# steineggerlab/unicore

Hardware: AMD Instinct MI355X
Metric: 3Di alignments/sec (cluster path) (higher is better)
Workload: dtype u16

## Files before the change

unicore_amd/csrc/uc_prefilter.hip:

```cpp
#include <hip/hip_runtime.h>

#include <algorithm>
#include <cstdlib>
#include <cstring>
#include <type_traits>

#include <rocprim/rocprim.hpp>

#include "uc_engine.h"

namespace uc {

constexpr uint32_t KMER_INVALID = 0xFFFFFFFFu;

struct KmerCfg {
    int koff[K];
    int span;
    int thr;
};

__device__ __forceinline__ uint32_t find_seq(const uint32_t *off, uint32_t lo, uint32_t hi, uint32_t p) {
    while (hi - lo > 1) {
        const uint32_t mid = lo + ((hi - lo) >> 1);
        if (off[mid] <= p) lo = mid; else hi = mid;
// ... 51 lines not shown
        bits[w] = m;
    }
}

constexpr int SIM_NEED_MAX = 49;
struct SimTables {
    int8_t sc[KA][KA];
    uint8_t ord[KA][KA];
    int8_t rowmax[KA];
    uint8_t lcnt[KA][2 * SIM_NEED_MAX + 1];
    uint32_t pmask[KA][KA + 1];
};

__device__ void build_sim_tables(SimTables &t, const int8_t *S3) {
    for (int a = threadIdx.x; a < KA; a += blockDim.x) {
        int8_t sc[KA];
        uint8_t ord[KA];
        for (int b = 0; b < KA; b++) { sc[b] = S3[a * 21 + b]; ord[b] = (uint8_t)b; }
        for (int i = 1; i < KA; i++) {
            const int8_t s = sc[i];
            const uint8_t o = ord[i];
            int k = i - 1;
            while (k >= 0 && (sc[k] < s)) { sc[k + 1] = sc[k]; ord[k + 1] = ord[k]; k--; }
            sc[k + 1] = s;
            ord[k + 1] = o;
        }
        for (int b = 0; b < KA; b++) { t.sc[a][b] = sc[b]; t.ord[a][b] = ord[b]; }
        t.rowmax[a] = sc[0];
    }
    for (int i = threadIdx.x; i < KA * (2 * SIM_NEED_MAX + 1); i += blockDim.x) {
        const int a = i / (2 * SIM_NEED_MAX + 1), need = i % (2 * SIM_NEED_MAX + 1) - SIM_NEED_MAX;
        int n = 0;
        for (int b = 0; b < KA; b++) n += S3[a * 21 + b] >= need ? 1 : 0;
        t.lcnt[a][i % (2 * SIM_NEED_MAX + 1)] = (uint8_t)n;
    }
    __syncthreads();
    for (int i = threadIdx.x; i < KA * (KA + 1); i += blockDim.x) {
        const int a = i / (KA + 1), n = i % (KA + 1);
        uint32_t m = 0;
        for (int j = 0; j < n; j++) m |= 1u << t.ord[a][j];
        t.pmask[a][n] = m;
    }
// ... 1 lines not shown

__device__ __forceinline__ bool query_kmer_at(const DeviceDb &db, const KmerCfg &cfg, uint32_t qbegin, uint32_t qend,
                                              uint32_t p, uint32_t *q, uint32_t *i, uint32_t c[K]) {
    const uint32_t s = find_seq(db.off, qbegin, qend, p);
    const uint32_t j = p - db.off[s], len = db.len[s];
    *q = s;
    *i = j;
    if (!(j + cfg.span <= len && j <= 65535u)) return false;
    bool ok = true;
#pragma unroll
    for (int m = 0; m < K; m++) { c[m] = db.s3[p + cfg.koff[m]]; ok &= c[m] < KA; }
    return ok;
}

constexpr int RUN_STAGE = 256;

struct RunList {
    uint32_t *pidx;
    uint64_t *val;
    uint64_t cap;
};

constexpr int LEAFQ = 256;
constexpr int POSQ = 128;
constexpr int SIM_MIN_WAVE_POS = 256;
constexpr int SIM_MAX_BLOCKS = 1024;

__global__ void __launch_bounds__(256) sim_runs_kernel(const DeviceDb db, KmerCfg cfg, uint32_t qbegin, uint32_t qend,
                                                            uint32_t p0, uint32_t p1, const uint32_t *koff, RunList out,
                                                            unsigned long long *counters,
                                                            const uint32_t *dk ,
                                                            uint32_t *nsim_k ,
                                                            uint32_t item_stride ,
                                                            const uint32_t *kbits = nullptr ) {
    __shared__ SimTables tab;
    __shared__ uint32_t s_mul[K];
    __shared__ uint32_t s_n[4];
    __shared__ uint64_t s_val[4][RUN_STAGE];
    __shared__ uint32_t s_pi[4][RUN_STAGE];
    __shared__ uint32_t s_qv[4][LEAFQ], s_qp[4][LEAFQ], s_qm[4][LEAFQ];
    __shared__ uint32_t s_pc[4][POSQ], s_pp[4][POSQ];
    __shared__ uint64_t s_pr[4][POSQ];
    build_sim_tables(tab, db.S3);
    const int wv = threadIdx.x >> 6, lane = threadIdx.x & 63;
    if (threadIdx.x < K) { uint32_t m = 1; for (int i = 0; i < K - 1 - (int)threadIdx.x; i++) m *= KA; s_mul[threadIdx.x] = m; }
    if (lane == 0) s_n[wv] = 0;
    __syncthreads();
    volatile uint32_t *vn = &s_n[wv];
    volatile uint64_t *vval = s_val[wv];
    volatile uint32_t *vpi = s_pi[wv];
    volatile uint32_t *qv = s_qv[wv], *qp = s_qp[wv], *qm = s_qm[wv];
    volatile uint32_t *pc = s_pc[wv], *pp = s_pp[wv];
    volatile uint64_t *pr = s_pr[wv];
    const int thr = cfg.thr, thrb = thr + 256;

    auto flush_runs = [&]() {
        const uint32_t n = *vn;
        uint32_t blo = 0, bhi = 0;
        if (lane == 0) {
            const unsigned long long b = atomicAdd(counters + 3, (unsigned long long)n);
            blo = (uint32_t)b; bhi = (uint32_t)(b >> 32);
        }
        blo = (uint32_t)__shfl((int)blo, 0, 64);
        bhi = (uint32_t)__shfl((int)bhi, 0, 64);
        const uint64_t base = ((uint64_t)bhi << 32) | blo;
        for (uint32_t k = lane; k < n; k += 64) {
            const uint64_t w = base + k;
            if (w < out.cap) { out.pidx[w] = vpi[k]; out.val[w] = vval[k]; }
        }
        __builtin_amdgcn_wave_barrier();
        if (lane == 0) *vn = 0;
        __builtin_amdgcn_wave_barrier();
    };
    unsigned long long nhit = 0;
    auto drain_leaves = [&](uint32_t qn) {
        for (uint32_t b = 0; b < qn; b += 64) {
            const uint32_t i = b + lane;
            uint32_t m = 0, v0 = 0, pi = 0;
            if (i < qn) {
                v0 = qv[i]; pi = qp[i]; m = qm[i];
                if (kbits) {
                    const uint32_t w = v0 >> 5, sh = v0 & 31;
                    const uint64_t two = (uint64_t)kbits[w] | ((uint64_t)(sh > 32 - KA ? kbits[w + 1] : 0u) << 32);
// ... 136 lines not shown
            }
            const uint64_t lm = __builtin_amdgcn_ballot_w64(leaf);
            if (lm) {
                if (leaf) { const uint32_t slot = qn + (uint32_t)__popcll(lm & ((1ull << lane) - 1ull)); qv[slot] = leafv; qp[slot] = pidx; qm[slot] = leafm; }
                qn += (uint32_t)__popcll(lm);
                nsim += (unsigned long long)__popc(leafm);
                if (qn > LEAFQ - 64) { __builtin_amdgcn_wave_barrier(); drain_leaves(qn); qn = 0; }
            }
        }
        __builtin_amdgcn_wave_barrier();
        drain_leaves(qn);
        if (nsim_k && has_item) nsim_k[pidx] = lc;
    }
    __builtin_amdgcn_wave_barrier();
    flush_runs();
    for (int o = 32; o > 0; o >>= 1) { nsim += __shfl_down(nsim, o, 64); nhit += __shfl_down(nhit, o, 64); }
    if (lane == 0) {
        if (nsim) atomicAdd(counters + 0, nsim);
        if (nhit) atomicAdd(counters + 4, nhit);
    }
}

__global__ void __launch_bounds__(256) query_kmer_kernel(const DeviceDb db, KmerCfg cfg, uint32_t qbegin, uint32_t qend, uint32_t p0, uint32_t p1,
                                                         uint32_t *qk, uint8_t *flag) {
    for (uint64_t idx = (uint64_t)blockIdx.x * 256 + threadIdx.x; idx < p1 - p0; idx += (uint64_t)gridDim.x * 256) {
        uint32_t q, i, c[K];
        uint32_t key = KMER_INVALID;
        if (query_kmer_at(db, cfg, qbegin, qend, p0 + (uint32_t)idx, &q, &i, c)) {
            uint32_t v = 0, mul = 1;
#pragma unroll
            for (int m = 0; m < K; m++) { v += c[m] * mul; mul *= KA; }
            key = v;
            flag[v] = 1;
// ... 170 lines not shown
        const uint32_t want = db.off[qbegin + i] - p0;
        uint64_t lo = 0, hi = n_runs;
        while (lo < hi) { const uint64_t m = (lo + hi) >> 1; if (rpidx[m] < want) lo = m + 1; else hi = m; }
        qr[i] = lo;
    }
}

__global__ void __launch_bounds__(256) run_order_key_kernel(uint32_t nq, const uint64_t *qr, uint32_t *key, uint32_t *idx) {
    for (uint32_t i = blockIdx.x * 256 + threadIdx.x; i < nq; i += gridDim.x * 256) {
        const uint64_t c = qr[i + 1] - qr[i];
        key[i] = 0xFFFFFFFFu - (uint32_t)min<uint64_t>(c, 0xFFFFFFFFull);
        idx[i] = i;
    }
}

template <bool C> struct TdType { using type = uint64_t; };
template <> struct TdType<true> { using type = uint32_t; };

template <bool C>
__global__ void __launch_bounds__(FT) filter_kernel(const DeviceDb db, uint32_t qbegin, uint32_t p0, const uint32_t *rpidx,
                                                    const uint64_t *rval, const uint64_t *qr, const uint32_t *order, const void *ent, KeyFmt fmt,
                                                    unsigned long long *region_cursor, void *region_v, uint64_t region_cap,
                                                    uint64_t *qbase, uint32_t *qsurv) {
    using TD = typename TdType<C>::type;
    struct __attribute__((aligned(4))) TD4 { TD v[KPT]; };
    TD *region = (TD *)region_v;
    extern __shared__ __attribute__((aligned(16))) uint32_t f_lds[];
    constexpr int BW = 1 << (FB_LOG2 - 5);
    constexpr int RPT = FILTER_RPT;
    constexpr int TR = RPT * FT;
    uint32_t *B1 = f_lds, *B2 = f_lds + BW;
    uint2 *s_run = (uint2 *)(f_lds + 2 * BW);
    uint32_t *s_pref = (uint32_t *)(s_run + TR);
    uint32_t *s_wsum = s_pref + TR + 1;
    uint64_t *s_misc = (uint64_t *)(((uintptr_t)(s_wsum + 16) + 7) & ~(uintptr_t)7);
    const int tid = threadIdx.x, lane = tid & 63, wv = tid >> 6;
    const uint32_t qi = order[blockIdx.x];
// ... 82 lines not shown
    };
    auto mark1 = [&](uint64_t td) {
        uint32_t g;
        const uint32_t h = slot_of(td, g), bit = 1u << (h & 31), gbit = 1u << (g & 31);
        const uint32_t old = atomicOr(&B1[h >> 5], bit);
        if (old & bit) atomicOr(&B2[h >> 5], bit);
        const uint32_t gold = atomicOr(&B1[g >> 5], gbit);
        if (gold & gbit) atomicOr(&B2[g >> 5], gbit);
    };
    auto twice1 = [&](uint64_t td) -> uint32_t {
        uint32_t g;
        const uint32_t h = slot_of(td, g);
        return ((B2[h >> 5] >> (h & 31)) & (B2[g >> 5] >> (g & 31))) & 1u;
    };

    {
        uint64_t part = 0;
        for (uint64_t r = r0 + tid; r < r1; r += FT) part += rval[r] >> 32;
        for (int o = 32; o > 0; o >>= 1) part += __shfl_down(part, o, 64);
        uint64_t *s_part = (uint64_t *)s_pref;
        if (lane == 0) s_part[wv] = part;
        __syncthreads();
        if (tid == 0) {
            uint64_t tot = 0;
            for (int w = 0; w < FT / 64; w++) tot += s_part[w];
            s_misc[2] = atomicAdd(region_cursor, (unsigned long long)((tot + KPT - 1) / KPT * KPT));
            ((uint32_t *)&s_misc[3])[0] = 0;
            ((uint32_t *)&s_misc[3])[1] = 0;
        }
        __syncthreads();
    }
    const uint64_t base = s_misc[2];
    uint32_t *cur = (uint32_t *)&s_misc[3];
    uint32_t total = 0;
    prefetch_tile(r0);
    for (uint64_t tile = r0; tile < r1; tile += TR) {
        load_tile(tile);
        prefetch_tile(tile + TR);
        const uint32_t T = s_pref[TR];
        using ET = typename std::conditional<C, uint32_t, uint64_t>::type;
        auto mark_store = [&](TD4 &td, int n, uint32_t k4) {
#pragma unroll
            for (int i = 0; i < KPT; i++) {
                if (i >= n) { td.v[i] = td.v[0]; continue; }
                mark1(td.v[i]);
            }
            const uint64_t w = base + total + k4;
            if (n && w + KPT <= region_cap) {
                if (n == KPT) *(TD4 *)(region + w) = td;
                else {
#pragma unroll
                    for (int i = 0; i < KPT; i++) if (i < n) region[w + i] = td.v[i];
                }
            }
        };
        for (uint32_t k4 = (uint32_t)KPT * tid; k4 < T; k4 += 2u * KPT * FT) {
            const uint32_t k4b = k4 + (uint32_t)KPT * FT;
            uint32_t ia[KPT], ib[KPT];
            int32_t sa[KPT], sb[KPT];
            const int na = locate(k4, T, ia, sa);
            const int nb = locate(k4b < T ? k4b : k4, T, ib, sb);
            ET ea[KPT], eb[KPT];
            gather(ia, ea);
            gather(ib, eb);
            TD4 ta, tb;
            to_td(ea, sa, ta.v);
            mark_store(ta, na, k4);
            to_td(eb, sb, tb.v);
            mark_store(tb, k4b < T ? nb : 0, k4b);
        }
        total += T;
        __syncthreads();
    }
    __threadfence_block();
    __syncthreads();
    const uint32_t n0 = (uint32_t)min<uint64_t>(total, region_cap > base ? region_cap - base : 0);
    const uint32_t n0r = n0;
    for (uint32_t k4 = (uint32_t)KPT * tid; k4 < n0r; k4 += 2u * KPT * FT) {
        TD4 td[2] = {};
        int nn[2];
#pragma unroll
        for (int g2 = 0; g2 < 2; g2++) {
            const uint32_t k = k4 + (uint32_t)g2 * KPT * FT;
            nn[g2] = k >= n0 ? 0 : (n0 - k < (uint32_t)KPT ? (int)(n0 - k) : KPT);
            if (nn[g2] == KPT) td[g2] = *(const TD4 *)(region + base + k);
            else {
#pragma unroll
                for (int i = 0; i < KPT; i++) if (i < nn[g2]) td[g2].v[i] = region[base + k + i];
            }
        }
        uint32_t keep = 0;
// ... 553 lines not shown
        }
    }
}
__global__ void __launch_bounds__(256) owner_gather_kernel(uint64_t n, const uint32_t *idx, const uint32_t *hq, const uint32_t *ht, const int32_t *hs,
                                                           const int32_t *hd, uint32_t *oq, uint32_t *ot, int32_t *os, int32_t *od) {
    for (uint64_t i = (uint64_t)blockIdx.x * 256 + threadIdx.x; i < n; i += (uint64_t)gridDim.x * 256) {
        const uint32_t j = idx[i];
        oq[i] = hq[j]; ot[i] = ht[j]; os[i] = hs[j]; od[i] = hd[j];
    }
}

struct WidenU32 {
    __host__ __device__ uint64_t operator()(uint32_t x) const { return (uint64_t)x; }
};

struct PrefilterScratch {
    DevBuf<unsigned long long> d_counters;
    DevBuf<char> d_temp;
    DevBuf<uint32_t> d_koff, k_in, k_out, d_ent32, v_in32, d_okey, d_okey2, d_oidx, d_order;
    DevBuf<uint64_t> d_ent, v_in;
    DevBuf<uint32_t> d_cnt, d_flag, d_cq, d_ct, d_rpidx2, d_qsurv;
    DevBuf<uint32_t> d_qcand, d_qmir, d_qrec;
    DevBuf<uint64_t> d_coff;
    DevBuf<uint64_t> d_keys, d_keys2, d_pos, d_skey, d_skey2, d_rval2, d_qbase, d_soff, d_qr;
    DevBuf<int32_t> d_cd, d_cd2, d_score, d_mval;
    DevBuf<uint64_t> d_mkey;
    DevBuf<uint32_t> acc_q, acc_t, pass_q, pass_t;
    DevBuf<int32_t> acc_s, acc_d, pass_s, pass_d;
    DevBuf<uint8_t> d_kflag, d_wflag;
    DevBuf<uint32_t> d_qk, d_kid, d_dk, d_nsimk, d_drk, d_drk2, d_roff, d_nr, d_src, d_ph;
    DevBuf<uint64_t> d_drv, d_drv2, d_cumh, d_cumr, d_qh, d_qrn;
    DevBuf<RankRec> d_rec;
    DevBuf<uint32_t> d_kbits;
    UngappedAllWork ua;
    template <class F> void each(F f) {
        f(d_counters); f(d_temp); f(d_koff); f(k_in); f(k_out); f(d_ent32); f(v_in32); f(d_okey); f(d_okey2); f(d_oidx); f(d_order);
        f(d_ent); f(v_in); f(d_cnt); f(d_flag); f(d_cq); f(d_ct); f(d_rpidx2); f(d_qsurv); f(d_keys); f(d_keys2); f(d_pos); f(d_skey);
        f(d_skey2); f(d_rval2); f(d_qbase); f(d_soff); f(d_qr); f(d_cd); f(d_cd2); f(d_score); f(d_kflag); f(d_wflag); f(d_qk); f(d_kid); f(d_dk);
        f(d_nsimk); f(d_drk); f(d_drk2); f(d_roff); f(d_nr); f(d_src); f(d_ph); f(d_drv); f(d_drv2); f(d_cumh); f(d_cumr); f(d_qh); f(d_qrn); f(d_rec); f(d_kbits); f(d_mkey); f(d_mval); f(acc_q); f(acc_t); f(pass_q); f(pass_t); f(acc_s); f(acc_d); f(pass_s); f(pass_d);
        f(d_qcand); f(d_qmir); f(d_qrec); f(d_coff); f(ua.score); f(ua.diag); f(ua.pairs); f(ua.prof); f(ua.prof_off);
    }
    size_t bytes() {
        size_t b = 0;
        each([&](auto &x) { b += x.cap * sizeof(*x.p); });
        return b;
    }
    void release_bytes(size_t target) {
        if (getenv("UC_TIMING")) {
            fprintf(stderr, "unicore-cluster[timing]: prefilter scratch %.1f GiB, %.1f GiB to give back before the gapped stage; buffers >= 2 GiB (index in PrefilterScratch::each: GiB):", bytes() / 1073741824.0, target / 1073741824.0);
            int i = 0;
            each([&](auto &x) { const double g = x.cap * sizeof(*x.p) / 1073741824.0; if (g >= 2.0) fprintf(stderr, " %d:%.1f", i, g); i++; });
            fprintf(stderr, "\n");
        }
        if (!target) return;
        if (target >= bytes()) { each([&](auto &x) { if (x.cap * sizeof(*x.p) >= ((size_t)1 << 30)) x.release(); }); return; }
// ... 45 lines not shown
    if (hit_off[n] != n_hits) fail(UC_ERR_GENERIC, "%s: hit list bookkeeping mismatch", who);
}

constexpr uint64_t RUN_MAX = 1ull << 29;
struct PrefilterPass {
    KmerCfg cfg;
    KeyFmt fmt;
    uint32_t tbegin = 0, tend = 0;
    uint32_t qbegin = 0, qend = 0;
    uint32_t mirror_q0 = UINT32_MAX;
    bool count_sims = false;
    double density_limit = 0.0, *density_out = nullptr;
    const void *ent_p = nullptr;
    uint32_t n_entries = 0;
    uint64_t HIT_CAP = 0, HIT_CAP_BIG = 0, DRUN_MAX = 0;
    uint64_t td_queries = 0, td_keys = 0, filt_queries = 0, filt_keys = 0;
    uint32_t td_cap = 0;
    uint64_t n_hits_total = 0, n_cand_total = 0, cand_cap = 0, run_cap = 1ull << 20;
    double t_kmer = 0, t_ung = 0, t_sel = 0, gpu_ms = 0;
};
struct SuperBatch {
    uint32_t begin = 0, end = 0;
    uint32_t P0 = 0, NP = 0;
    std::vector<uint64_t> h_qh, h_qr;
    uint64_t hit_cap = 0;
    double frac = 1.0;
};
struct QueryBatch {
    uint32_t qa = 0, qb = 0;
    uint64_t total_hits = 0, n_runs = 0;
// ... 43 lines not shown
    S.d_kbits.reserve((KSPACE + 31) / 32);
    hipLaunchKernelGGL(kmer_bits_kernel, grid_for((KSPACE + 31) / 32), dim3(256), 0, E.stream, (const uint32_t *)S.d_koff.p, S.d_kbits.p);
    UC_HIP(hipMemcpyAsync(&PP.n_entries, S.d_koff.p + KSPACE, 4, hipMemcpyDeviceToHost, E.stream));
    UC_HIP(hipStreamSynchronize(E.stream));
    UC_HIP(hipGetLastError());
    PP.gpu_ms = E.timed_ms_end();
    E.stats.n_index_entries += PP.n_entries;
    E.stats.algorithmic_bytes[UC_ST_INDEX] += 6ull * PP.n_entries + 8ull * KSPACE;
    E.stats.stage_seconds[UC_ST_INDEX] += t_index.seconds();
}

static dim3 sim_grid(uint64_t items) {
    return dim3((uint32_t)std::min<uint64_t>(std::max<uint64_t>(1, (items + 4 * SIM_MIN_WAVE_POS - 1) / (4 * SIM_MIN_WAVE_POS)), SIM_MAX_BLOCKS));
}

static uint64_t distinct_runs(Engine &E, PrefilterPass &PP, const SuperBatch &SB, uint32_t nd, uint64_t &n_druns, uint64_t &drun_cap) {
    PrefilterScratch &S = *E.pre;
    const uint32_t nqa = SB.end - SB.begin;
    if (nqa > 1 && nd > (1u << 16)) {
        const uint32_t st = 64;
        UC_HIP(hipMemsetAsync(S.d_counters.p + 3, 0, 32, E.stream));
        UC_HIP(hipMemsetAsync(S.d_counters.p, 0, 8, E.stream));
        hipLaunchKernelGGL(sim_runs_kernel, sim_grid((nd + st - 1) / st), dim3(256), 0, E.stream, E.ddb, PP.cfg, 0u, 0u, 0u, nd, S.d_koff.p, RunList{nullptr, nullptr, 0},
                           S.d_counters.p, S.d_dk.p, (uint32_t *)nullptr, st, (const uint32_t *)S.d_kbits.p);
        unsigned long long c5[5];
        UC_HIP(hipMemcpyAsync(c5, S.d_counters.p, 40, hipMemcpyDeviceToHost, E.stream));
        UC_HIP(hipStreamSynchronize(E.stream));
        if ((double)c5[3] * st > 0.9 * (double)PP.DRUN_MAX) return (uint64_t)((double)c5[3] * st / 0.9);
    }
    n_druns = 0; drun_cap = S.d_drk.cap;
    for (;;) {
        drun_cap = std::min<uint64_t>(1ull << 32, std::max<uint64_t>(drun_cap, std::max<uint64_t>(1u << 20, std::min<uint64_t>(PP.DRUN_MAX, (uint64_t)nd * 16))));
        S.d_drk.reserve(drun_cap); S.d_drv.reserve(drun_cap);
        UC_HIP(hipMemsetAsync(S.d_counters.p + 3, 0, 32, E.stream));
        UC_HIP(hipMemsetAsync(S.d_counters.p, 0, 8, E.stream));
        const RunList rl{S.d_drk.p, S.d_drv.p, drun_cap};
        hipLaunchKernelGGL(sim_runs_kernel, sim_grid(nd), dim3(256), 0, E.stream, E.ddb, PP.cfg, 0u, 0u, 0u, nd, S.d_koff.p, rl, S.d_counters.p, S.d_dk.p, S.d_nsimk.p, 1u,
                           (const uint32_t *)S.d_kbits.p);
        unsigned long long c5[5];
        UC_HIP(hipMemcpyAsync(c5, S.d_counters.p, 40, hipMemcpyDeviceToHost, E.stream));
        UC_HIP(hipStreamSynchronize(E.stream));
        n_druns = c5[3];
        if (getenv("UC_TIMING")) fprintf(stderr, "unicore-cluster[timing]: similar k-mers of %u distinct k-mers: %llu index runs\n", nd, (unsigned long long)n_druns);
        if (n_druns > PP.DRUN_MAX && nqa > 1) return n_druns;
        if (n_druns > drun_cap) {
            if (n_druns >= (1ull << 32)) fail(UC_ERR_GENERIC, "%u distinct k-mers of query %u produce %llu index ranges", nd, SB.begin, (unsigned long long)n_druns);
            drun_cap = n_druns;
            UC_HIP(hipMemsetAsync(S.d_nsimk.p, 0, (size_t)std::max<uint32_t>(nd, 1) * 4, E.stream));
            continue;
        }
        return 0;
    }
}

enum class PlanStatus { planned, too_dense , too_many_runs  };
struct PlanResult { PlanStatus status; uint64_t over_runs; };
static PlanResult plan_superbatch(Engine &E, PrefilterPass &PP, SuperBatch &SB, uint32_t sa, uint32_t sb) {
    PrefilterScratch &S = *E.pre;
    uint64_t plan_hits = 0;
    SB.begin = sa; SB.end = sb;
    SB.P0 = E.h_poff[sa]; SB.NP = E.h_poff[sb] - SB.P0;
    const uint32_t NP = SB.NP, nqa = sb - sa;
    Timer t_p;
    E.timed_ms_begin();
    S.d_qk.reserve((size_t)NP + 1); S.d_kflag.reserve((size_t)KSPACE + 1); S.d_kid.reserve((size_t)KSPACE + 1);
    UC_HIP(hipMemsetAsync(S.d_kflag.p, 0, (size_t)KSPACE + 1, E.stream));
    hipLaunchKernelGGL(query_kmer_kernel, grid_for(NP), dim3(256), 0, E.stream, E.ddb, PP.cfg, sa, sb, SB.P0, SB.P0 + NP, S.d_qk.p, S.d_kflag.p);
    auto fin = rocprim::make_transform_iterator(S.d_kflag.p, FlagToU32());
    rocprim_call(S.d_temp, [&](void *t, size_t &b) { return rocprim::exclusive_scan(t, b, fin, S.d_kid.p, 0u, (size_t)KSPACE + 1, rocprim::plus<uint32_t>(), E.stream); });
    uint32_t nd = 0;
    UC_HIP(hipMemcpyAsync(&nd, S.d_kid.p + KSPACE, 4, hipMemcpyDeviceToHost, E.stream));
    UC_HIP(hipStreamSynchronize(E.stream));
    S.d_dk.reserve(std::max<uint32_t>(nd, 1)); S.d_nsimk.reserve(std::max<uint32_t>(nd, 1));
    UC_HIP(hipMemsetAsync(S.d_nsimk.p, 0, (size_t)std::max<uint32_t>(nd, 1) * 4, E.stream));
    hipLaunchKernelGGL(distinct_kmer_kernel, grid_for(KSPACE), dim3(256), 0, E.stream, S.d_kflag.p, S.d_kid.p, S.d_dk.p);
    uint64_t n_druns = 0, drun_cap = 0;
    if (const uint64_t over_runs = distinct_runs(E, PP, SB, nd, n_druns, drun_cap)) {
        PP.gpu_ms += E.timed_ms_end();
        PP.t_kmer += t_p.seconds();
        return {PlanStatus::too_many_runs, over_runs};
    }
    unsigned dbits = 1;
    while ((1ull << dbits) < nd) dbits++;
    S.d_drk2.reserve(drun_cap); S.d_drv2.reserve(drun_cap);
    if (n_druns)
        rocprim_call(S.d_temp, [&](void *t, size_t &b) { return rocprim::radix_sort_pairs(t, b, S.d_drk.p, S.d_drk2.p, S.d_drv.p, S.d_drv2.p, (size_t)n_druns, 0u, dbits, E.stream); });
    S.d_roff.reserve((size_t)nd + 1); S.d_rec.reserve(std::max<uint32_t>(nd, 1));
    hipLaunchKernelGGL(rank_offsets_kernel, grid_for((uint64_t)nd + 1), dim3(256), 0, E.stream, S.d_drk2.p, (uint32_t)n_druns, nd, S.d_roff.p);
    if (nd) hipLaunchKernelGGL(rank_rec_kernel, grid_for(nd), dim3(256), 0, E.stream, S.d_roff.p, S.d_drv2.p, S.d_nsimk.p, nd, S.d_rec.p);
    S.d_nr.reserve((size_t)NP + 1); S.d_src.reserve((size_t)NP + 1); S.d_ph.reserve((size_t)NP + 1);
    S.d_cumh.reserve((size_t)NP + 1); S.d_cumr.reserve((size_t)NP + 1);
    UC_HIP(hipMemsetAsync(S.d_counters.p, 0, 8, E.stream));
    UC_HIP(hipMemsetAsync(S.d_nr.p + NP, 0, 4, E.stream));
    UC_HIP(hipMemsetAsync(S.d_ph.p + NP, 0, 4, E.stream));
    hipLaunchKernelGGL(position_runs_kernel, grid_for(NP, E.count_grid_cap), dim3(256), 0, E.stream, S.d_qk.p, NP, S.d_kid.p, S.d_rec.p, S.d_nr.p, S.d_src.p, S.d_ph.p, S.d_counters.p);
    auto hin = rocprim::make_transform_iterator(S.d_ph.p, WidenU32());
    auto rin = rocprim::make_transform_iterator(S.d_nr.p, WidenU32());
    rocprim_call(S.d_temp, [&](void *t, size_t &b) { return rocprim::exclusive_scan(t, b, hin, S.d_cumh.p, (uint64_t)0, (size_t)NP + 1, rocprim::plus<uint64_t>(), E.stream); });
    rocprim_call(S.d_temp, [&](void *t, size_t &b) { return rocprim::exclusive_scan(t, b, rin, S.d_cumr.p, (uint64_t)0, (size_t)NP + 1, rocprim::plus<uint64_t>(), E.stream); });
    S.d_qh.reserve(nqa); S.d_qrn.reserve(nqa);
    hipLaunchKernelGGL(query_totals_kernel, grid_for(nqa), dim3(256), 0, E.stream, E.ddb.off, sa, nqa, SB.P0, S.d_cumh.p, S.d_cumr.p, S.d_qh.p, S.d_qrn.p);
// ... 63 lines not shown
    B.kbits = (unsigned)(PP.fmt.dbits + PP.fmt.tbits) + qbits;
    return B;
}

static uint64_t compact_u64(Engine &E, DevBuf<char> &tmp, uint32_t *cnt, uint64_t *pos, uint64_t n, const uint32_t *also = nullptr, uint32_t *also_out = nullptr) {
    auto in = rocprim::make_transform_iterator(cnt, WidenU32());
    rocprim_call(tmp, [&](void *t, size_t &b) { return rocprim::exclusive_scan(t, b, in, pos, (uint64_t)0, (size_t)n, rocprim::plus<uint64_t>(), E.stream); });
    uint64_t lp = 0; uint32_t lc = 0;
    UC_HIP(hipMemcpyAsync(&lp, pos + (n - 1), 8, hipMemcpyDeviceToHost, E.stream));
    UC_HIP(hipMemcpyAsync(&lc, cnt + (n - 1), 4, hipMemcpyDeviceToHost, E.stream));
    if (also) UC_HIP(hipMemcpyAsync(also_out, also, 4, hipMemcpyDeviceToHost, E.stream));
    UC_HIP(hipStreamSynchronize(E.stream));
    return lp + lc;
}

static void expand_keys_filtered(Engine &E, PrefilterPass &PP, QueryBatch &B) {
    PrefilterScratch &S = *E.pre;
    const KeyFmt &fmt = PP.fmt;
    const uint32_t qa = B.qa, qp0 = B.qp0, nq = B.qb - B.qa;
    S.d_qbase.reserve(nq); S.d_qsurv.reserve(nq); S.d_soff.reserve((size_t)nq + 1);
    const uint64_t region_cap = B.total_hits + (uint64_t)KPT * nq;
    S.d_keys.reserve(fmt.compact ? region_cap : 2 * region_cap);
    S.d_qr.reserve((size_t)nq + 1);
    hipLaunchKernelGGL(run_range_kernel, grid_for((uint64_t)nq + 1), dim3(256), 0, E.stream, E.ddb, qa, nq, qp0, S.d_rpidx2.p, B.n_runs, S.d_qr.p);
    S.d_okey.reserve(nq); S.d_okey2.reserve(nq); S.d_oidx.reserve(nq); S.d_order.reserve(nq);
    hipLaunchKernelGGL(run_order_key_kernel, grid_for(nq), dim3(256), 0, E.stream, nq, S.d_qr.p, S.d_okey.p, S.d_oidx.p);
    rocprim_call(S.d_temp, [&](void *t, size_t &b) { return rocprim::radix_sort_pairs(t, b, S.d_okey.p, S.d_okey2.p, S.d_oidx.p, S.d_order.p, (size_t)nq, 0u, 32u, E.stream); });
    auto launch = [&](auto kern) {
        static PerDeviceOnce once[2];
        once[fmt.compact ? 1 : 0]([&] { UC_HIP(hipFuncSetAttribute((const void *)kern, hipFuncAttributeMaxDynamicSharedMemorySize, (int)filter_lds(FILTER_RPT))); });
        hipLaunchKernelGGL(kern, dim3(nq), dim3(FT), filter_lds(FILTER_RPT), E.stream, E.ddb, qa, qp0, S.d_rpidx2.p, S.d_rval2.p, S.d_qr.p, S.d_order.p, PP.ent_p, fmt,
                           S.d_counters.p + 5, (void *)S.d_keys.p, region_cap, S.d_qbase.p, S.d_qsurv.p);
    };
    if (fmt.compact) launch(filter_kernel<true>);
    else launch(filter_kernel<false>);
    unsigned long long taken = 0;
    uint32_t last_rec = 0;
    const bool onchip = fmt.compact && PP.td_cap > 0;
    if (onchip) {
        int rbits = 1;
        while ((1ull << rbits) < (uint64_t)std::max<uint32_t>(PP.tend - PP.tbegin, 1)) rbits++;
        S.d_qcand.reserve(nq); S.d_qmir.reserve(nq); S.d_qrec.reserve(nq); S.d_coff.reserve(nq);
        UC_HIP(hipMemsetAsync(S.d_counters.p + 7, 0, 8, E.stream));
        hipLaunchKernelGGL(td_select_kernel<false>, dim3(nq), dim3(TDS_T), 0, E.stream, (uint32_t *)S.d_keys.p, S.d_qbase.p, S.d_qsurv.p, S.d_order.p, qa, PP.mirror_q0,
                           E.p.min_diag_hits, fmt.dbits, (unsigned)std::min(32, rbits + fmt.dbits), PP.td_cap, S.d_qcand.p, S.d_qmir.p, S.d_qrec.p, S.d_counters.p + 7);
        if (PP.td_cap > (uint32_t)TDS_SMALL_IPT * TDS_T)
            hipLaunchKernelGGL(td_select_kernel<true>, dim3(nq), dim3(TDS_T), 0, E.stream, (uint32_t *)S.d_keys.p, S.d_qbase.p, S.d_qsurv.p, S.d_order.p, qa, PP.mirror_q0,
// ... 117 lines not shown

static bool prefilter_one(Engine &E, uint32_t tbegin, uint32_t tend, uint32_t qbegin, uint32_t qend, bool count_sims, double density_limit,
                          double *density_out, uint32_t mirror_q0) {
    UC_HIP(hipSetDevice(E.device));
    const uint32_t n = E.hdb.n;
    PrefilterPass PP;
    for (int m = 0; m < K; m++) PP.cfg.koff[m] = E.p.koff[m];
    PP.cfg.span = E.p.span; PP.cfg.thr = E.p.kmer_thr;
    PP.tbegin = tbegin; PP.tend = tend; PP.qbegin = qbegin; PP.qend = qend; PP.mirror_q0 = mirror_q0;
    PP.count_sims = count_sims; PP.density_limit = density_limit; PP.density_out = density_out;
    const char *hc = getenv("UC_HIT_CAP");
    PP.HIT_CAP = hc ? std::max<uint64_t>(1u << 20, strtoull(hc, nullptr, 10)) : (3ull << 29);
    PP.HIT_CAP_BIG = hc ? PP.HIT_CAP : (15ull << 28);
    const char *dm = getenv("UC_DRUN_MAX");
    PP.DRUN_MAX = dm ? std::max<uint64_t>(1, strtoull(dm, nullptr, 10)) : (1ull << 31);
    const char *to = getenv("UC_TD_ONCHIP"), *tc = getenv("UC_TD_ONCHIP_CAP");
    PP.td_cap = to && atoi(to) == 0 ? 0u : TDS_CAP;
    if (PP.td_cap && tc) {
        const uint64_t want = strtoull(tc, nullptr, 10);
        uint32_t c = 64;
        while (c < TDS_CAP && 2ull * c <= want) c *= 2;
        PP.td_cap = c;
    }

    E.hit_cnt.assign(n, 0);
    E.hit_off.assign((size_t)n + 1, 0);
    E.n_hits = 0;
    E.alns_valid = false;
    E.clear_edges();
    const uint64_t sims_before = E.stats.n_sim_kmers;

    if (n > (1u << 24)) fail(UC_ERR_GENERIC, "prefilter: %u sequences exceed the 2^24 limit of the hit keys", n);
    if (!E.pre) E.pre = ParkedScratch<PrefilterScratch>::take_or_new(E.device);
    E.pre->d_counters.reserve(8);
    UC_HIP(hipMemsetAsync(E.pre->d_counters.p, 0, 64, E.stream));

    build_index(E, PP);
    SuperBatch SB;
    SB.begin = SB.end = qbegin;
    for (uint32_t qa = qbegin; qa < qend;) {
        if (qa >= SB.end && !choose_superbatch(E, PP, SB, qa)) return false;
        Timer t_b;
        E.timed_ms_begin();
        QueryBatch B = cut_batch(E, PP, SB, qa);
        uint64_t n_cand = 0;
        if (B.total_hits) {
            if (E.p.min_diag_hits >= 2 && B.total_hits < (1ull << 32)) expand_keys_filtered(E, PP, B);
            else expand_keys_plain(E, PP, B);
            n_cand = select_diagonals(E, PP, B);
        }
        UC_HIP(hipGetLastError());
        PP.gpu_ms += E.timed_ms_end();
        PP.t_kmer += t_b.seconds();
        PP.n_cand_total += n_cand;
        if (n_cand) {
            rescore_ungapped(E, PP, n_cand);
            select_and_append(E, PP, n_cand);
        }
        qa = B.qb;
    }
    finish_chunk(E, PP, sims_before);
    return true;
// ... 20 lines not shown
            acc_n = E.merge_hits_dev(acc_n, S.acc_q.p, S.acc_t.p, S.acc_s.p, S.acc_d.p, n_pass, S.pass_q.p, S.pass_t.p, S.pass_s.p, S.pass_d.p, !mir, 0, 1);
            if (c + 1 == chunks.size()) installed = true;
            else swap_acc();
        }
    }
    if (!installed) E.merge_hits_dev(acc_n, S.acc_q.p, S.acc_t.p, S.acc_s.p, S.acc_d.p, 0, nullptr, nullptr, nullptr, nullptr, true, 0, 1);
    return true;
}

static void prefilter_exhaustive(Engine &E, uint32_t tbegin, uint32_t tend, uint32_t qbegin, uint32_t qend) {
    UC_HIP(hipSetDevice(E.device));
    if (E.hdb.n > (1u << 24)) fail(UC_ERR_GENERIC, "prefilter: %u sequences exceed the 2^24 limit of the hit keys", E.hdb.n);
    logf(3, "unicore-cluster: --prefilter-mode 1: all %u x %u pairs are scored on every diagonal; --k-score, --min-diag-hits and -s have no effect\n", qend - qbegin, tend - tbegin);
    if (!E.pre) E.pre = ParkedScratch<PrefilterScratch>::take_or_new(E.device);
    PrefilterScratch &S = *E.pre;
    S.d_counters.reserve(8);
    UC_HIP(hipMemsetAsync(S.d_counters.p, 0, 64, E.stream));
    uint64_t budget = UNGAPPED_ALL_TILE_BYTES;
    if (const char *ev = getenv("UC_UNGAPPED_TILE_BYTES")) budget = std::max<uint64_t>(1, strtoull(ev, nullptr, 10));
    uint32_t QB = 1, TC = 1;
    ungapped_all_plan(budget, qend - qbegin, tend - tbegin, &QB, &TC);
    UngappedAllWork &W = S.ua;
    PrefilterPass PP;
    bool installed = false;
    const auto swap_acc = [&] { swap_hits(E, S.acc_q, S.acc_t, S.acc_s, S.acc_d); };
    uint64_t acc_n = 0, cells = 0;
    for (uint32_t qa = qbegin; qa < qend; qa += std::min(QB, qend - qa))
        for (uint32_t ta = tbegin; ta < tend; ta += std::min(TC, tend - ta)) {
            const uint32_t nq = std::min(QB, qend - qa), nt = std::min(TC, tend - ta);
            const uint64_t np = (uint64_t)nq * nt;
            Timer t_u;
            E.timed_ms_begin();
// ... 246 lines not shown
```

Baseline: 23.05 million.

## Reserve run slots in per-wave chunks and precompute filter region bases by scan

sim_runs_kernel now reserves output slots for similar-k-mer runs in fixed-size chunks per wave instead of one global atomic per flush, and pads unused chunk tails with sentinel entries. Run and nsim counts are moved to separate counters, and the sort uses the extended slot count. filter_kernel no longer does a block reduction plus a global atomic to claim its region; base offsets come from an exclusive scan over per-query hit counts. This cuts contention on global atomics, at the cost of larger run buffers and extra padding entries to sort.

```diff
diff --git a/unicore_amd/csrc/uc_prefilter.hip b/unicore_amd/csrc/uc_prefilter.hip
--- a/unicore_amd/csrc/uc_prefilter.hip
+++ b/unicore_amd/csrc/uc_prefilter.hip
@@ -89,8 +89,8 @@
 
 __device__ void build_sim_tables(SimTables &t, const int8_t *S3) {
     for (int a = threadIdx.x; a < KA; a += blockDim.x) {
-        int8_t sc[KA];
-        uint8_t ord[KA];
+        int8_t *sc = t.sc[a];
+        uint8_t *ord = t.ord[a];
         for (int b = 0; b < KA; b++) { sc[b] = S3[a * 21 + b]; ord[b] = (uint8_t)b; }
         for (int i = 1; i < KA; i++) {
             const int8_t s = sc[i];
@@ -100,7 +100,6 @@
             sc[k + 1] = s;
             ord[k + 1] = o;
         }
-        for (int b = 0; b < KA; b++) { t.sc[a][b] = sc[b]; t.ord[a][b] = ord[b]; }
         t.rowmax[a] = sc[0];
     }
     for (int i = threadIdx.x; i < KA * (2 * SIM_NEED_MAX + 1); i += blockDim.x) {
@@ -132,6 +131,7 @@
 }
 
 constexpr int RUN_STAGE = 256;
+constexpr uint32_t RUN_CHUNK = 2048;
 
 struct RunList {
     uint32_t *pidx;
@@ -150,6 +150,7 @@
                                                             const uint32_t *dk ,
                                                             uint32_t *nsim_k ,
                                                             uint32_t item_stride ,
+                                                            uint32_t run_chunk ,
                                                             const uint32_t *kbits = nullptr ) {
     __shared__ SimTables tab;
     __shared__ uint32_t s_mul[K];
@@ -172,19 +173,30 @@
     volatile uint64_t *pr = s_pr[wv];
     const int thr = cfg.thr, thrb = thr + 256;
 
+    uint64_t cpos = 0, cend = 0, nruns = 0;
     auto flush_runs = [&]() {
-        const uint32_t n = *vn;
-        uint32_t blo = 0, bhi = 0;
-        if (lane == 0) {
-            const unsigned long long b = atomicAdd(counters + 3, (unsigned long long)n);
-            blo = (uint32_t)b; bhi = (uint32_t)(b >> 32);
-        }
-        blo = (uint32_t)__shfl((int)blo, 0, 64);
-        bhi = (uint32_t)__shfl((int)bhi, 0, 64);
-        const uint64_t base = ((uint64_t)bhi << 32) | blo;
-        for (uint32_t k = lane; k < n; k += 64) {
-            const uint64_t w = base + k;
-            if (w < out.cap) { out.pidx[w] = vpi[k]; out.val[w] = vval[k]; }
+        const uint32_t n = (uint32_t)__builtin_amdgcn_readfirstlane((int)*vn);
+        nruns += n;
+        if (out.pidx) {
+            for (uint32_t k0 = 0; k0 < n;) {
+                if (cpos == cend) {
+                    uint32_t blo = 0, bhi = 0;
+                    if (lane == 0) {
+                        const unsigned long long b = atomicAdd(counters + 8, (unsigned long long)run_chunk);
+                        blo = (uint32_t)b; bhi = (uint32_t)(b >> 32);
+                    }
+                    blo = (uint32_t)__builtin_amdgcn_readfirstlane((int)blo);
+                    bhi = (uint32_t)__builtin_amdgcn_readfirstlane((int)bhi);
+                    cpos = ((uint64_t)bhi << 32) | blo;
+                    cend = cpos + run_chunk;
+                }
+                const uint32_t m = (uint32_t)min((uint64_t)(n - k0), cend - cpos);
+                for (uint32_t k = lane; k < m; k += 64) {
+                    const uint64_t w = cpos + k;
+                    if (w < out.cap) { out.pidx[w] = vpi[k0 + k]; out.val[w] = vval[k0 + k]; }
+                }
+                cpos += m; k0 += m;
+            }
         }
         __builtin_amdgcn_wave_barrier();
         if (lane == 0) *vn = 0;
@@ -351,9 +363,11 @@
     }
     __builtin_amdgcn_wave_barrier();
     flush_runs();
+    for (uint64_t w = cpos + lane; w < min(cend, out.cap); w += 64) { out.pidx[w] = p1 - p0; out.val[w] = 0; }
     for (int o = 32; o > 0; o >>= 1) { nsim += __shfl_down(nsim, o, 64); nhit += __shfl_down(nhit, o, 64); }
     if (lane == 0) {
-        if (nsim) atomicAdd(counters + 0, nsim);
+        if (nruns) atomicAdd(counters + 3, (unsigned long long)nruns);
+        if (nsim) atomicAdd(counters + 9, nsim);
         if (nhit) atomicAdd(counters + 4, nhit);
     }
 }
@@ -554,13 +568,18 @@
     }
 }
 
+struct RoundUpKpt {
+    __host__ __device__ uint64_t operator()(uint64_t h) const { return (h + KPT - 1) / KPT * KPT; }
+};
+
 template <bool C> struct TdType { using type = uint64_t; };
 template <> struct TdType<true> { using type = uint32_t; };
 
 template <bool C>
 __global__ void __launch_bounds__(FT) filter_kernel(const DeviceDb db, uint32_t qbegin, uint32_t p0, const uint32_t *rpidx,
                                                     const uint64_t *rval, const uint64_t *qr, const uint32_t *order, const void *ent, KeyFmt fmt,
-                                                    unsigned long long *region_cursor, void *region_v, uint64_t region_cap,
+                                                    const uint64_t *rbase ,
+                                                    const uint64_t *qhits , void *region_v, uint64_t region_cap,
                                                     uint64_t *qbase, uint32_t *qsurv) {
     using TD = typename TdType<C>::type;
     struct __attribute__((aligned(4))) TD4 { TD v[KPT]; };
@@ -673,24 +692,10 @@
         return ((B2[h >> 5] >> (h & 31)) & (B2[g >> 5] >> (g & 31))) & 1u;
     };
 
-    {
-        uint64_t part = 0;
-        for (uint64_t r = r0 + tid; r < r1; r += FT) part += rval[r] >> 32;
-        for (int o = 32; o > 0; o >>= 1) part += __shfl_down(part, o, 64);
-        uint64_t *s_part = (uint64_t *)s_pref;
-        if (lane == 0) s_part[wv] = part;
-        __syncthreads();
-        if (tid == 0) {
-            uint64_t tot = 0;
-            for (int w = 0; w < FT / 64; w++) tot += s_part[w];
-            s_misc[2] = atomicAdd(region_cursor, (unsigned long long)((tot + KPT - 1) / KPT * KPT));
-            ((uint32_t *)&s_misc[3])[0] = 0;
-            ((uint32_t *)&s_misc[3])[1] = 0;
-        }
-        __syncthreads();
-    }
-    const uint64_t base = s_misc[2];
+    const uint64_t base = rbase[qi];
+    const uint64_t region_end = min(base + (qhits[qi] + KPT - 1) / KPT * KPT, region_cap);
     uint32_t *cur = (uint32_t *)&s_misc[3];
+    if (tid == 0) { cur[0] = 0; cur[1] = 0; }
     uint32_t total = 0;
     prefetch_tile(r0);
     for (uint64_t tile = r0; tile < r1; tile += TR) {
@@ -705,7 +710,7 @@
                 mark1(td.v[i]);
             }
             const uint64_t w = base + total + k4;
-            if (n && w + KPT <= region_cap) {
+            if (n && w + n <= region_end) {
                 if (n == KPT) *(TD4 *)(region + w) = td;
                 else {
 #pragma unroll
@@ -733,7 +738,7 @@
     }
     __threadfence_block();
     __syncthreads();
-    const uint32_t n0 = (uint32_t)min<uint64_t>(total, region_cap > base ? region_cap - base : 0);
+    const uint32_t n0 = (uint32_t)min<uint64_t>(total, region_end > base ? region_end - base : 0);
     const uint32_t n0r = n0;
     for (uint32_t k4 = (uint32_t)KPT * tid; k4 < n0r; k4 += 2u * KPT * FT) {
         TD4 td[2] = {};
@@ -1317,6 +1322,7 @@
     __host__ __device__ uint64_t operator()(uint32_t x) const { return (uint64_t)x; }
 };
 
+constexpr size_t PREFILTER_COUNTERS = 10;
 struct PrefilterScratch {
     DevBuf<unsigned long long> d_counters;
     DevBuf<char> d_temp;
@@ -1325,7 +1331,7 @@
     DevBuf<uint32_t> d_cnt, d_flag, d_cq, d_ct, d_rpidx2, d_qsurv;
     DevBuf<uint32_t> d_qcand, d_qmir, d_qrec;
     DevBuf<uint64_t> d_coff;
-    DevBuf<uint64_t> d_keys, d_keys2, d_pos, d_skey, d_skey2, d_rval2, d_qbase, d_soff, d_qr;
+    DevBuf<uint64_t> d_keys, d_keys2, d_pos, d_skey, d_skey2, d_rval2, d_qbase, d_soff, d_qr, d_rbase;
     DevBuf<int32_t> d_cd, d_cd2, d_score, d_mval;
     DevBuf<uint64_t> d_mkey;
     DevBuf<uint32_t> acc_q, acc_t, pass_q, pass_t;
@@ -1341,7 +1347,7 @@
         f(d_ent); f(v_in); f(d_cnt); f(d_flag); f(d_cq); f(d_ct); f(d_rpidx2); f(d_qsurv); f(d_keys); f(d_keys2); f(d_pos); f(d_skey);
         f(d_skey2); f(d_rval2); f(d_qbase); f(d_soff); f(d_qr); f(d_cd); f(d_cd2); f(d_score); f(d_kflag); f(d_wflag); f(d_qk); f(d_kid); f(d_dk);
         f(d_nsimk); f(d_drk); f(d_drk2); f(d_roff); f(d_nr); f(d_src); f(d_ph); f(d_drv); f(d_drv2); f(d_cumh); f(d_cumr); f(d_qh); f(d_qrn); f(d_rec); f(d_kbits); f(d_mkey); f(d_mval); f(acc_q); f(acc_t); f(pass_q); f(pass_t); f(acc_s); f(acc_d); f(pass_s); f(pass_d);
-        f(d_qcand); f(d_qmir); f(d_qrec); f(d_coff); f(ua.score); f(ua.diag); f(ua.pairs); f(ua.prof); f(ua.prof_off);
+        f(d_qcand); f(d_qmir); f(d_qrec); f(d_coff); f(d_rbase); f(ua.score); f(ua.diag); f(ua.pairs); f(ua.prof); f(ua.prof_off);
     }
     size_t bytes() {
         size_t b = 0;
@@ -1417,6 +1423,8 @@
     const void *ent_p = nullptr;
     uint32_t n_entries = 0;
     uint64_t HIT_CAP = 0, HIT_CAP_BIG = 0, DRUN_MAX = 0;
+    uint64_t DRUN_CAP0 = 0;
+    uint32_t run_chunk = RUN_CHUNK;
     uint64_t td_queries = 0, td_keys = 0, filt_queries = 0, filt_keys = 0;
     uint32_t td_cap = 0;
     uint64_t n_hits_total = 0, n_cand_total = 0, cand_cap = 0, run_cap = 1ull << 20;
@@ -1490,38 +1498,42 @@
     return dim3((uint32_t)std::min<uint64_t>(std::max<uint64_t>(1, (items + 4 * SIM_MIN_WAVE_POS - 1) / (4 * SIM_MIN_WAVE_POS)), SIM_MAX_BLOCKS));
 }
 
-static uint64_t distinct_runs(Engine &E, PrefilterPass &PP, const SuperBatch &SB, uint32_t nd, uint64_t &n_druns, uint64_t &drun_cap) {
+static uint64_t distinct_runs(Engine &E, PrefilterPass &PP, const SuperBatch &SB, uint32_t nd, uint64_t &n_druns, uint64_t &n_ext, uint64_t &drun_cap) {
     PrefilterScratch &S = *E.pre;
     const uint32_t nqa = SB.end - SB.begin;
+    unsigned long long c[6];
     if (nqa > 1 && nd > (1u << 16)) {
         const uint32_t st = 64;
-        UC_HIP(hipMemsetAsync(S.d_counters.p + 3, 0, 32, E.stream));
-        UC_HIP(hipMemsetAsync(S.d_counters.p, 0, 8, E.stream));
+        UC_HIP(hipMemsetAsync(S.d_counters.p + 3, 0, 56, E.stream));
         hipLaunchKernelGGL(sim_runs_kernel, sim_grid((nd + st - 1) / st), dim3(256), 0, E.stream, E.ddb, PP.cfg, 0u, 0u, 0u, nd, S.d_koff.p, RunList{nullptr, nullptr, 0},
-                           S.d_counters.p, S.d_dk.p, (uint32_t *)nullptr, st, (const uint32_t *)S.d_kbits.p);
-        unsigned long long c5[5];
-        UC_HIP(hipMemcpyAsync(c5, S.d_counters.p, 40, hipMemcpyDeviceToHost, E.stream));
+                           S.d_counters.p, S.d_dk.p, (uint32_t *)nullptr, st, PP.run_chunk, (const uint32_t *)S.d_kbits.p);
+        UC_HIP(hipMemcpyAsync(c, S.d_counters.p + 3, 8, hipMemcpyDeviceToHost, E.stream));
         UC_HIP(hipStreamSynchronize(E.stream));
-        if ((double)c5[3] * st > 0.9 * (double)PP.DRUN_MAX) return (uint64_t)((double)c5[3] * st / 0.9);
-    }
-    n_druns = 0; drun_cap = S.d_drk.cap;
+        if ((double)c[0] * st > 0.9 * (double)PP.DRUN_MAX) return (uint64_t)((double)c[0] * st / 0.9);
+    }
+    const dim3 grid = sim_grid(nd);
+    const uint64_t tails = (uint64_t)grid.x * 4 * PP.run_chunk;
+    n_druns = n_ext = 0;
+    drun_cap = PP.DRUN_CAP0 ? PP.DRUN_CAP0
+                            : std::max<uint64_t>(S.d_drk.cap, std::max<uint64_t>(1u << 20, std::min<uint64_t>(PP.DRUN_MAX, (uint64_t)nd * 16) + tails));
     for (;;) {
-        drun_cap = std::min<uint64_t>(1ull << 32, std::max<uint64_t>(drun_cap, std::max<uint64_t>(1u << 20, std::min<uint64_t>(PP.DRUN_MAX, (uint64_t)nd * 16))));
+        drun_cap = std::min<uint64_t>(1ull << 32, drun_cap);
         S.d_drk.reserve(drun_cap); S.d_drv.reserve(drun_cap);
-        UC_HIP(hipMemsetAsync(S.d_counters.p + 3, 0, 32, E.stream));
-        UC_HIP(hipMemsetAsync(S.d_counters.p, 0, 8, E.stream));
+        UC_HIP(hipMemsetAsync(S.d_counters.p + 3, 0, 56, E.stream));
         const RunList rl{S.d_drk.p, S.d_drv.p, drun_cap};
-        hipLaunchKernelGGL(sim_runs_kernel, sim_grid(nd), dim3(256), 0, E.stream, E.ddb, PP.cfg, 0u, 0u, 0u, nd, S.d_koff.p, rl, S.d_counters.p, S.d_dk.p, S.d_nsimk.p, 1u,
-                           (const uint32_t *)S.d_kbits.p);
-        unsigned long long c5[5];
-        UC_HIP(hipMemcpyAsync(c5, S.d_counters.p, 40, hipMemcpyDeviceToHost, E.stream));
+        hipLaunchKernelGGL(sim_runs_kernel, grid, dim3(256), 0, E.stream, E.ddb, PP.cfg, 0u, 0u, 0u, nd, S.d_koff.p, rl, S.d_counters.p, S.d_dk.p, S.d_nsimk.p, 1u,
+                           PP.run_chunk, (const uint32_t *)S.d_kbits.p);
+        UC_HIP(hipMemcpyAsync(c, S.d_counters.p + 3, 48, hipMemcpyDeviceToHost, E.stream));
         UC_HIP(hipStreamSynchronize(E.stream));
-        n_druns = c5[3];
-        if (getenv("UC_TIMING")) fprintf(stderr, "unicore-cluster[timing]: similar k-mers of %u distinct k-mers: %llu index runs\n", nd, (unsigned long long)n_druns);
+        n_druns = c[0]; n_ext = c[5];
+        if (getenv("UC_TIMING"))
+            fprintf(stderr, "unicore-cluster[timing]: similar k-mers of %u distinct k-mers: %llu index runs in %llu reserved slots (capacity %llu)\n", nd,
+                    (unsigned long long)n_druns, (unsigned long long)n_ext, (unsigned long long)drun_cap);
         if (n_druns > PP.DRUN_MAX && nqa > 1) return n_druns;
-        if (n_druns > drun_cap) {
-            if (n_druns >= (1ull << 32)) fail(UC_ERR_GENERIC, "%u distinct k-mers of query %u produce %llu index ranges", nd, SB.begin, (unsigned long long)n_druns);
-            drun_cap = n_druns;
+        if (n_ext > drun_cap) {
+            if (n_druns >= (1ull << 32) || n_ext >= (1ull << 32))
+                fail(UC_ERR_GENERIC, "%u distinct k-mers of query %u produce %llu index ranges", nd, SB.begin, (unsigned long long)n_druns);
+            drun_cap = n_ext;
             UC_HIP(hipMemsetAsync(S.d_nsimk.p, 0, (size_t)std::max<uint32_t>(nd, 1) * 4, E.stream));
             continue;
         }
@@ -1550,17 +1562,17 @@
     S.d_dk.reserve(std::max<uint32_t>(nd, 1)); S.d_nsimk.reserve(std::max<uint32_t>(nd, 1));
     UC_HIP(hipMemsetAsync(S.d_nsimk.p, 0, (size_t)std::max<uint32_t>(nd, 1) * 4, E.stream));
     hipLaunchKernelGGL(distinct_kmer_kernel, grid_for(KSPACE), dim3(256), 0, E.stream, S.d_kflag.p, S.d_kid.p, S.d_dk.p);
-    uint64_t n_druns = 0, drun_cap = 0;
-    if (const uint64_t over_runs = distinct_runs(E, PP, SB, nd, n_druns, drun_cap)) {
+    uint64_t n_druns = 0, n_ext = 0, drun_cap = 0;
+    if (const uint64_t over_runs = distinct_runs(E, PP, SB, nd, n_druns, n_ext, drun_cap)) {
         PP.gpu_ms += E.timed_ms_end();
         PP.t_kmer += t_p.seconds();
         return {PlanStatus::too_many_runs, over_runs};
     }
     unsigned dbits = 1;
-    while ((1ull << dbits) < nd) dbits++;
+    while ((1ull << dbits) <= nd) dbits++;
     S.d_drk2.reserve(drun_cap); S.d_drv2.reserve(drun_cap);
     if (n_druns)
-        rocprim_call(S.d_temp, [&](void *t, size_t &b) { return rocprim::radix_sort_pairs(t, b, S.d_drk.p, S.d_drk2.p, S.d_drv.p, S.d_drv2.p, (size_t)n_druns, 0u, dbits, E.stream); });
+        rocprim_call(S.d_temp, [&](void *t, size_t &b) { return rocprim::radix_sort_pairs(t, b, S.d_drk.p, S.d_drk2.p, S.d_drv.p, S.d_drv2.p, (size_t)n_ext, 0u, dbits, E.stream); });
     S.d_roff.reserve((size_t)nd + 1); S.d_rec.reserve(std::max<uint32_t>(nd, 1));
     hipLaunchKernelGGL(rank_offsets_kernel, grid_for((uint64_t)nd + 1), dim3(256), 0, E.stream, S.d_drk2.p, (uint32_t)n_druns, nd, S.d_roff.p);
     if (nd) hipLaunchKernelGGL(rank_rec_kernel, grid_for(nd), dim3(256), 0, E.stream, S.d_roff.p, S.d_drv2.p, S.d_nsimk.p, nd, S.d_rec.p);
@@ -1654,13 +1666,17 @@
     return lp + lc;
 }
 
-static void expand_keys_filtered(Engine &E, PrefilterPass &PP, QueryBatch &B) {
+static void expand_keys_filtered(Engine &E, PrefilterPass &PP, const SuperBatch &SB, QueryBatch &B) {
     PrefilterScratch &S = *E.pre;
     const KeyFmt &fmt = PP.fmt;
     const uint32_t qa = B.qa, qp0 = B.qp0, nq = B.qb - B.qa;
     S.d_qbase.reserve(nq); S.d_qsurv.reserve(nq); S.d_soff.reserve((size_t)nq + 1);
     const uint64_t region_cap = B.total_hits + (uint64_t)KPT * nq;
     S.d_keys.reserve(fmt.compact ? region_cap : 2 * region_cap);
+    S.d_rbase.reserve(nq);
+    const uint64_t *qhits = S.d_qh.p + (qa - SB.begin);
+    auto kin = rocprim::make_transform_iterator(qhits, RoundUpKpt());
+    rocprim_call(S.d_temp, [&](void *t, size_t &b) { return rocprim::exclusive_scan(t, b, kin, S.d_rbase.p, (uint64_t)0, (size_t)nq, rocprim::plus<uint64_t>(), E.stream); });
     S.d_qr.reserve((size_t)nq + 1);
     hipLaunchKernelGGL(run_range_kernel, grid_for((uint64_t)nq + 1), dim3(256), 0, E.stream, E.ddb, qa, nq, qp0, S.d_rpidx2.p, B.n_runs, S.d_qr.p);
     S.d_okey.reserve(nq); S.d_okey2.reserve(nq); S.d_oidx.reserve(nq); S.d_order.reserve(nq);
@@ -1670,7 +1686,7 @@
         static PerDeviceOnce once[2];
         once[fmt.compact ? 1 : 0]([&] { UC_HIP(hipFuncSetAttribute((const void *)kern, hipFuncAttributeMaxDynamicSharedMemorySize, (int)filter_lds(FILTER_RPT))); });
         hipLaunchKernelGGL(kern, dim3(nq), dim3(FT), filter_lds(FILTER_RPT), E.stream, E.ddb, qa, qp0, S.d_rpidx2.p, S.d_rval2.p, S.d_qr.p, S.d_order.p, PP.ent_p, fmt,
-                           S.d_counters.p + 5, (void *)S.d_keys.p, region_cap, S.d_qbase.p, S.d_qsurv.p);
+                           (const uint64_t *)S.d_rbase.p, qhits, (void *)S.d_keys.p, region_cap, S.d_qbase.p, S.d_qsurv.p);
     };
     if (fmt.compact) launch(filter_kernel<true>);
     else launch(filter_kernel<false>);
@@ -1818,6 +1834,8 @@
     PP.HIT_CAP_BIG = hc ? PP.HIT_CAP : (15ull << 28);
     const char *dm = getenv("UC_DRUN_MAX");
     PP.DRUN_MAX = dm ? std::max<uint64_t>(1, strtoull(dm, nullptr, 10)) : (1ull << 31);
+    if (const char *rc = getenv("UC_RUN_CHUNK")) PP.run_chunk = (uint32_t)std::min<uint64_t>(1u << 20, std::max<uint64_t>(64, strtoull(rc, nullptr, 10)));
+    if (const char *c0 = getenv("UC_DRUN_CAP0")) PP.DRUN_CAP0 = std::max<uint64_t>(1, strtoull(c0, nullptr, 10));
     const char *to = getenv("UC_TD_ONCHIP"), *tc = getenv("UC_TD_ONCHIP_CAP");
     PP.td_cap = to && atoi(to) == 0 ? 0u : TDS_CAP;
     if (PP.td_cap && tc) {
@@ -1836,8 +1854,8 @@
 
     if (n > (1u << 24)) fail(UC_ERR_GENERIC, "prefilter: %u sequences exceed the 2^24 limit of the hit keys", n);
     if (!E.pre) E.pre = ParkedScratch<PrefilterScratch>::take_or_new(E.device);
-    E.pre->d_counters.reserve(8);
-    UC_HIP(hipMemsetAsync(E.pre->d_counters.p, 0, 64, E.stream));
+    E.pre->d_counters.reserve(PREFILTER_COUNTERS);
+    UC_HIP(hipMemsetAsync(E.pre->d_counters.p, 0, PREFILTER_COUNTERS * 8, E.stream));
 
     build_index(E, PP);
     SuperBatch SB;
@@ -1849,7 +1867,7 @@
         QueryBatch B = cut_batch(E, PP, SB, qa);
         uint64_t n_cand = 0;
         if (B.total_hits) {
-            if (E.p.min_diag_hits >= 2 && B.total_hits < (1ull << 32)) expand_keys_filtered(E, PP, B);
+            if (E.p.min_diag_hits >= 2 && B.total_hits < (1ull << 32)) expand_keys_filtered(E, PP, SB, B);
             else expand_keys_plain(E, PP, B);
             n_cand = select_diagonals(E, PP, B);
         }
@@ -1900,8 +1918,8 @@
     logf(3, "unicore-cluster: --prefilter-mode 1: all %u x %u pairs are scored on every diagonal; --k-score, --min-diag-hits and -s have no effect\n", qend - qbegin, tend - tbegin);
     if (!E.pre) E.pre = ParkedScratch<PrefilterScratch>::take_or_new(E.device);
     PrefilterScratch &S = *E.pre;
-    S.d_counters.reserve(8);
-    UC_HIP(hipMemsetAsync(S.d_counters.p, 0, 64, E.stream));
+    S.d_counters.reserve(PREFILTER_COUNTERS);
+    UC_HIP(hipMemsetAsync(S.d_counters.p, 0, PREFILTER_COUNTERS * 8, E.stream));
     uint64_t budget = UNGAPPED_ALL_TILE_BYTES;
     if (const char *ev = getenv("UC_UNGAPPED_TILE_BYTES")) budget = std::max<uint64_t>(1, strtoull(ev, nullptr, 10));
     uint32_t QB = 1, TC = 1;
```

After: 23.14 million, median of 6. No clear change (+0.4%).
